# run-house/kubetorch

Hardware: AMD Instinct MI355X
Metric: llama3_8b_ddp_bf16_tokens_per_sec (higher is better)
Workload: dtype bf16; 1 GPU; model=llama3-8b, global_batch=4, seq_len=4096, parallelism=dp1

## Files before the change

kubetorch_amd/models/llama.py:

```python
from dataclasses import dataclass

import torch
import torch.nn as nn
import torch.nn.functional as F

from kubetorch_amd import ops


@dataclass
class LlamaConfig:
    dim: int = 4096
    n_layers: int = 32
    n_heads: int = 32
    n_kv_heads: int = 8
    intermediate: int = 14336
    vocab_size: int = 128256
    max_seq_len: int = 8192
    rope_base: float = 500000.0
    norm_eps: float = 1e-5
    init_std: float = 0.02

    @property
    def head_dim(self):
        return self.dim // self.n_heads
# ... 57 lines not shown
        if P == 0:
            o = layer.attn._sdpa(q, kf, vf, causal=True)
        elif S == 1:
            o = layer.attn._sdpa(q, kf, vf)
        else:
            L = P + S
            ar = torch.arange(L, device=q.device)
            mask = (ar.view(1, L) <= (P + torch.arange(
                S, device=q.device)).view(S, 1)).view(1, 1, S, L)
            o = layer.attn._sdpa(q, kf, vf, mask=mask)
        return o.transpose(1, 2).reshape(B, S, -1)


class RMSNorm(nn.Module):
    def __init__(self, dim, eps):
        super().__init__()
        self.weight = nn.Parameter(torch.ones(dim))
        self.eps = eps

    def forward(self, x):
        return ops.rmsnorm(x, self.weight, self.eps)


class Attention(nn.Module):
    def __init__(self, cfg: LlamaConfig):
        super().__init__()
        self.cfg = cfg
        d, hd = cfg.dim, cfg.head_dim
        self.n_heads, self.n_kv = cfg.n_heads, cfg.n_kv_heads
        self.wqkv = ops.Linear(d, (cfg.n_heads + 2 * cfg.n_kv_heads) * hd, bias=False)
        self.wo = ops.Linear(cfg.n_heads * hd, d, bias=False)

    def _sdpa(self, q, k, v, causal=False, mask=None):
        kw = dict(attn_mask=mask, is_causal=causal)
        if self.n_kv != self.n_heads:
            try:
                return F.scaled_dot_product_attention(
                    q, k, v, enable_gqa=True, **kw)
            except (TypeError, RuntimeError):
                rep = self.n_heads // self.n_kv
                k = k.repeat_interleave(rep, dim=1)
                v = v.repeat_interleave(rep, dim=1)
        return F.scaled_dot_product_attention(q, k, v, **kw)

    def forward(self, x, cos, sin):
        import os

        B, S, _ = x.shape
        hd = self.cfg.head_dim
        qkv = self.wqkv(x)
        q, k, v = qkv.split(
            [self.n_heads * hd, self.n_kv * hd, self.n_kv * hd], dim=-1
        )
        attn_impl = os.environ.get("KT_ATTN", "ck")
        use_v3 = (attn_impl == "ck"
                  and ops.flash_attention_v3_supported(S, hd, x.device, x.dtype))
        q_oscale = (hd ** -0.5) * ops.LOG2E if use_v3 else 1.0
        q = ops.rope(q.view(B, S, self.n_heads, hd), cos, sin, oscale=q_oscale)
        k = ops.rope(k.view(B, S, self.n_kv, hd), cos, sin)
        v = v.view(B, S, self.n_kv, hd)
        q, k, v = (t.transpose(1, 2) for t in (q, k, v))
        if use_v3:
            o = ops.flash_attention(q, k, v, impl="v3")
            return self.wo(o.transpose(1, 2).reshape(B, S, -1))
        if (attn_impl in ("ck", "custom")
                and ops.flash_attention_supported(q, k, v, True)):
            o = ops.flash_attention(
                q, k, v, impl="wmma" if attn_impl == "custom" else "ck")
            return self.wo(o.transpose(1, 2).reshape(B, S, -1))
        o = self._sdpa(q, k, v, causal=True)
        o = o.transpose(1, 2).reshape(B, S, -1)
        return self.wo(o)


class MLP(nn.Module):
    def __init__(self, cfg: LlamaConfig):
        super().__init__()
        self.w_gate_up = ops.Linear(cfg.dim, 2 * cfg.intermediate, bias=False)
        self.w_down = ops.Linear(cfg.intermediate, cfg.dim, bias=False)

    def forward(self, x):
        return self.w_down(ops.swiglu(self.w_gate_up(x)))


class Block(nn.Module):
    def __init__(self, cfg: LlamaConfig):
        super().__init__()
        self.attn_norm = RMSNorm(cfg.dim, cfg.norm_eps)
        self.attn = Attention(cfg)
        self.mlp_norm = RMSNorm(cfg.dim, cfg.norm_eps)
        self.mlp = MLP(cfg)

    def forward(self, x, cos, sin):
        x = x + self.attn(self.attn_norm(x), cos, sin)
        x = x + self.mlp(self.mlp_norm(x))
        return x


class Llama(nn.Module):
    def __init__(self, cfg: LlamaConfig):
        super().__init__()
        self.cfg = cfg
        self.embed = nn.Embedding(cfg.vocab_size, cfg.dim)
        self.layers = nn.ModuleList(Block(cfg) for _ in range(cfg.n_layers))
        self.norm = RMSNorm(cfg.dim, cfg.norm_eps)
        self.lm_head = ops.Linear(cfg.dim, cfg.vocab_size, bias=False)
        cos, sin = ops.precompute_rope(cfg.max_seq_len, cfg.head_dim, cfg.rope_base)
        self.register_buffer("rope_cos", cos, persistent=False)
        self.register_buffer("rope_sin", sin, persistent=False)
        self.gradient_checkpointing = False
        self.reset_parameters()

    def gradient_checkpointing_enable(self, enabled=True):
        self.gradient_checkpointing = enabled
        return self

    def _apply(self, fn, recurse=True):
        ret = super()._apply(fn, recurse)
        if self.rope_cos.dtype != torch.float32:
            cos, sin = ops.precompute_rope(
                self.cfg.max_seq_len, self.cfg.head_dim, self.cfg.rope_base,
# ... 115 lines not shown
```

kubetorch_amd/ops/__init__.py:

```python
import importlib.util
import os

import torch

_EXT = None
_EXT_ERR = None


def _ext():
    global _EXT, _EXT_ERR
    if _EXT is not None:
        return _EXT
    if _EXT_ERR is not None:
        raise _EXT_ERR
    so = os.path.join(os.path.dirname(__file__), "_hip_ops.so")
    if not os.path.exists(so):
        _EXT_ERR = RuntimeError(
            f"kubetorch_amd HIP extension not built: {so} missing. "
            "Run `python -m kubetorch_amd.ops.build` (gfx950)."
        )
        raise _EXT_ERR
    spec = importlib.util.spec_from_file_location("kubetorch_amd.ops._hip_ops", so)
    mod = importlib.util.module_from_spec(spec)
    try:
# ... 193 lines not shown
        du = do * g * sig
        return torch.cat([dg, du], dim=-1).to(gu.dtype)


def swiglu(gate_up):
    return _SwiGLU.apply(gate_up)


class _FusedCE(torch.autograd.Function):
    @staticmethod
    def forward(ctx, logits, targets, ignore_index):
        V = logits.shape[-1]
        flat = logits.reshape(-1, V)
        t = targets.reshape(-1)
        n_valid = (t != ignore_index).sum().clamp(min=1)
        if logits.is_cuda:
            loss = _ext().cross_entropy_fwd_(flat, t.contiguous(), 1.0, ignore_index)
            dlogits = flat
        else:
            lf = flat.float()
            logp = torch.log_softmax(lf, dim=-1)
            loss = torch.nn.functional.nll_loss(
                logp, t, reduction="none", ignore_index=ignore_index
            )
            dlogits = torch.softmax(lf, dim=-1)
            valid = (t != ignore_index).unsqueeze(-1)
            dlogits.scatter_add_(
                1, t.clamp(min=0).unsqueeze(1), -torch.ones_like(t, dtype=torch.float32).unsqueeze(1)
            )
            dlogits = torch.where(valid, dlogits, torch.zeros_like(dlogits)).to(logits.dtype)
        ctx.save_for_backward(dlogits, n_valid)
        ctx.shape = logits.shape
        return loss.sum() / n_valid.to(loss.dtype)

    @staticmethod
    def backward(ctx, gout):
        dlogits, n_valid = ctx.saved_tensors
        scale = (gout / n_valid).to(torch.float32)
        if dlogits.is_cuda:
            g = _ext().scale_bf16(dlogits, scale.reshape(1))
        else:
            g = (dlogits * scale).to(dlogits.dtype)
        return g.reshape(ctx.shape), None, None


def fused_cross_entropy(logits, targets, ignore_index=-100):
    return _FusedCE.apply(logits, targets, ignore_index)


_LN2 = 0.6931471805599453
LOG2E = 1.4426950408889634


class _FlashAttention(torch.autograd.Function):
    @staticmethod
    def forward(ctx, q, k, v, scale, impl):
        if impl == "v3":
            o, lse = _ext().attn_fwd_v3(q, k, v, scale, prescaled=True)
            scale = _LN2
        elif impl == "ck":
            o, lse = _ext().attn_fwd_ck_tr(q, k, v, scale)
        else:
            q, k, v = q.contiguous(), k.contiguous(), v.contiguous()
            o, lse = _ext().attn_fwd(q, k, v, scale)
        ctx.save_for_backward(q, k, v, o, lse)
        ctx.scale = scale
        return o

    @staticmethod
    def backward(ctx, grad_out):
        import os

        q, k, v, o, lse = ctx.saved_tensors
        B, Hq, S, D = q.shape
        Hkv = k.shape[1]
        g = Hq // Hkv
        if os.environ.get("KT_ATTN_BWD") == "ck" and S % 128 == 0:
            dq, dk_e, dv_e = _ext().attn_bwd_ck(
                grad_out.contiguous(), q.contiguous(), k.contiguous(),
                v.contiguous(), o.contiguous(), lse.contiguous(), ctx.scale)
            if g > 1:
                dk = dk_e.view(B, Hkv, g, S, D).sum(2)
                dv = dv_e.view(B, Hkv, g, S, D).sum(2)
            else:
                dk, dv = dk_e, dv_e
            return dq, dk, dv, None, None
        if g > 1:
            k_exp = k.repeat_interleave(g, dim=1)
            v_exp = v.repeat_interleave(g, dim=1)
        else:
            k_exp, v_exp = k, v
        seed = torch.zeros((), dtype=torch.long, device=q.device)
        offset = torch.zeros((), dtype=torch.long, device=q.device)
        dq, dk, dv, _ = torch.ops.aten._scaled_dot_product_efficient_attention_backward(
            grad_out.contiguous(), q, k_exp, v_exp, None, o, lse, seed, offset,
            0.0, [True, True, True, False], True, scale=ctx.scale,
        )
        if g > 1:
            dk = dk.view(B, Hkv, g, S, D).sum(2)
            dv = dv.view(B, Hkv, g, S, D).sum(2)
        return dq, dk, dv, None, None


def flash_attention(q, k, v, scale=None, impl="ck"):
    if scale is None:
        scale = q.shape[-1] ** -0.5
    return _FlashAttention.apply(q, k, v, scale, impl)


def flash_attention_supported(q, k, v, is_causal):
    return (is_causal and q.is_cuda and q.dtype == torch.bfloat16
            and q.shape[-1] == 128 and q.shape[2] % 128 == 0
            and q.shape[2] >= 256 and hip_available())


def flash_attention_v3_supported(S, head_dim, device, dtype):
    return (head_dim == 128 and S % 256 == 0 and S >= 256
            and device.type == "cuda" and dtype == torch.bfloat16
            and hip_available())


PAGED_PAGE_SIZES = (16, 32, 64)
PAGED_HEAD_DIMS = (64, 128)
PAGED_GROUPS = (1, 2, 4, 8)


def _no_grad_inputs(name, *tensors):
    if any(t.requires_grad for t in tensors):
        raise RuntimeError(f"{name} is inference-only: an input requires grad")


def _check_pools(k_pages, v_pages):
    if k_pages.dim() != 4 or v_pages.shape != k_pages.shape:
        raise ValueError("k_pages/v_pages must be equal-shaped "
                         "[num_pages, n_kv, page_size, hd]")
    if not (k_pages.is_contiguous() and v_pages.is_contiguous()):
        raise ValueError("k_pages/v_pages must be contiguous")
    if k_pages.shape[2] not in PAGED_PAGE_SIZES:
        raise ValueError(f"page_size must be one of {PAGED_PAGE_SIZES}")
    if k_pages.shape[3] not in PAGED_HEAD_DIMS:
        raise ValueError(f"head_dim must be one of {PAGED_HEAD_DIMS}")


def paged_kv_write(k_new, v_new, k_pages, v_pages, slot_mapping):
    _no_grad_inputs("paged_kv_write", k_new, v_new, k_pages, v_pages)
    if k_pages.is_cuda:
        _ext().paged_kv_write(k_new, v_new, k_pages, v_pages, slot_mapping)
        return
    _check_pools(k_pages, v_pages)
    P, Hkv, ps, hd = k_pages.shape
    if (k_new.shape != v_new.shape or k_new.dim() != 3
            or tuple(k_new.shape[1:]) != (Hkv, hd)):
        raise ValueError("k_new/v_new must be [T, n_kv, hd] matching the pool")
    if slot_mapping.dtype != torch.int32 or \
            tuple(slot_mapping.shape) != (k_new.shape[0],):
        raise ValueError("slot_mapping must be [T] int32")
    slots = slot_mapping.long()
    keep = (slots >= 0) & (slots < P * ps)
    page, off = slots[keep] // ps, slots[keep] % ps
    k_pages[page, :, off] = k_new[keep].to(k_pages.dtype)
    v_pages[page, :, off] = v_new[keep].to(v_pages.dtype)


_PAGED_TARGET_WORKGROUPS = 512
_PAGED_MIN_TOKENS_PER_SPLIT = 256
_PAGED_MAX_SPLITS = 32


def paged_num_splits(batch, n_kv, max_tokens):
    want = -(-_PAGED_TARGET_WORKGROUPS // max(1, batch * n_kv))
    cap = max(1, max_tokens // _PAGED_MIN_TOKENS_PER_SPLIT)
    return max(1, min(want, cap, _PAGED_MAX_SPLITS))
# ... 367 lines not shown
```

kubetorch_amd/ops/hip/bindings.cpp:

```cpp

#include <cmath>
#include <cstdlib>

#include <torch/extension.h>

#include <ATen/hip/impl/HIPGuardImplMasqueradingAsCUDA.h>
#include <ATen/hip/impl/HIPStreamMasqueradingAsCUDA.h>

extern "C" {
void kt_rmsnorm_fwd(const void* x, const void* res, const void* w, void* y,
                    void* s_out, void* invrms, int N, int H, float eps,
                    hipStream_t stream);
void kt_rmsnorm_bwd(const void* dy, const void* ds, const void* x,
                    const void* w, const void* invrms, void* dx,
                    void* dw_partial, void* dw, int P, int N, int H,
                    hipStream_t stream);
void kt_rope(const void* x, void* o, const void* cost, const void* sint,
             long total_quads, int S, int Hh, int D, long src_t_stride,
             long src_h_stride, float sign, float oscale, hipStream_t stream);
void kt_swiglu_fwd(const void* gu, void* out, long N, int I,
                   hipStream_t stream);
void kt_swiglu_bwd(const void* dout, const void* gu, void* dgu, long N, int I,
                   hipStream_t stream);
void kt_cross_entropy_fwd(void* logits, const void* targets, void* loss,
                          int N, int V, float scale, long ignore_index,
                          hipStream_t stream);
void kt_scale_bf16(const void* in, void* out, const void* scale, long n,
                   hipStream_t stream);
void kt_adamw(void* p, const void* g, void* m, void* v, long n, float lr,
              float beta1, float beta2, float eps, float wd, float bc1,
              float bc2, float grad_scale, hipStream_t stream);
void kt_attn_fwd(const void* q, const void* k, const void* v, void* o,
                 void* lse, int B, int Hq, int Hkv, int S, float scale,
                 hipStream_t stream);
void kt_attn_fwd_ck(const void* q, const void* k, const void* v, void* o,
                    void* lse, int B, int Hq, int Hkv, int S, float scale,
                    const long* strides, hipStream_t stream);
void kt_attn_fwd_ck_tr(const void* q, const void* k, const void* v, void* o,
                       void* lse, int B, int Hq, int Hkv, int S, float scale,
                       const long* strides, hipStream_t stream);
void kt_attn_fwd_v3(const void* q, const void* k, const void* v, void* o,
                    void* lse, int B, int Hq, int Hkv, int S, float scale,
                    const long* strides, hipStream_t stream);
void kt_pack_segments(const void* ptrs, const void* nbytes, const void* offs,
                      void* base, int nseg, long max_nbytes, int to_base,
                      hipStream_t stream);
void kt_transpose_bf16(const void* src, long src_stride, void* dst, long R,
                       long C, hipStream_t stream);
void kt_transpose_segments_bf16(const void* src, void* dst, const void* table,
                                int nseg, long max_tiles, hipStream_t stream);
void kt_attn_bwd_ck(const void* q, const void* k, const void* v,
                    const void* o, const void* do_, const void* lse, void* d,
                    void* dq_acc, void* dq, void* dk, void* dv, int B, int Hq,
                    int Hkv, int S, float scale, int mask_mode, int pipe,
                    hipStream_t stream);
void kt_paged_kv_write(const void* k_new, const void* v_new, void* k_pages,
                       void* v_pages, const void* slot_mapping, long T,
                       int Hkv, int hd, int page_size, long num_pages,
                       long k_st, long k_sh, long v_st, long v_sh,
                       hipStream_t stream);
int kt_paged_attention_decode(const void* q, const void* k_pages,
                              const void* v_pages, const void* block_table,
                              const void* seq_lens, void* out, void* po,
                              void* pm, void* pl, int B, int Hq, int Hkv,
                              int hd, int page_size, int num_pages,
                              int max_blocks, int num_splits, float scale,
                              hipStream_t stream);
int kt_paged_attention_prefill(const void* q, const void* k_pages,
                               const void* v_pages, const void* block_table,
                               const void* cu_q_lens, const void* seq_lens,
                               void* out, long T, long q_st, long q_sh, int B,
                               int Hq, int Hkv, int hd, int page_size,
// ... 47 lines not shown
  CHECK_BF16_CONTIG(dy);
  CHECK_BF16_CONTIG(x);
  CHECK_BF16_CONTIG(w);
  const int H = (int)x.size(-1);
  const long N = x.numel() / H;
  TORCH_CHECK(H % 8 == 0, "H must be a multiple of 8");
  TORCH_CHECK(w.numel() == H, "weight shape mismatch");
  TORCH_CHECK(dy.sizes() == x.sizes(), "dy shape mismatch");
  TORCH_CHECK(invrms.is_cuda() && invrms.scalar_type() == at::kFloat &&
                  invrms.is_contiguous() && invrms.numel() == N,
              "invrms must be N contiguous fp32 values on GPU");
  int lds_max = 0;
  TORCH_CHECK(hipDeviceGetAttribute(&lds_max,
                                    hipDeviceAttributeMaxSharedMemoryPerBlock,
                                    x.device().index()) == hipSuccess,
              "cannot read the LDS limit");
  TORCH_CHECK((size_t)H * sizeof(float) + 64 <= (size_t)lds_max,
              "H too large for the rmsnorm_bwd LDS accumulator");
  c10::hip::OptionalHIPGuardMasqueradingAsCUDA guard(x.device());
  auto dx = at::empty_like(x);
  auto dw = at::empty_like(w);
  const int P = N < 512 ? (int)N : 512;
  auto dw_partial = at::empty({P, H}, x.options().dtype(at::kFloat));
  const void* ds_ptr = nullptr;
  if (ds.has_value()) {
    CHECK_BF16_CONTIG(ds.value());
    TORCH_CHECK(ds->sizes() == x.sizes(), "ds shape mismatch");
    ds_ptr = ds->data_ptr();
  }
  kt_rmsnorm_bwd(dy.data_ptr(), ds_ptr, x.data_ptr(), w.data_ptr(),
                 invrms.data_ptr(), dx.data_ptr(), dw_partial.data_ptr(),
                 dw.data_ptr(), P, (int)N, H, cur_stream(x));
  return {dx, dw};
}

at::Tensor rope(const at::Tensor& x, const at::Tensor& cost,
                const at::Tensor& sint, int64_t S, double sign,
                double oscale) {
  TORCH_CHECK(x.is_cuda() && x.scalar_type() == at::kBFloat16);
  TORCH_CHECK(x.dim() == 3, "rope expects [T, Hh, D]");
  TORCH_CHECK(x.stride(2) == 1, "head dim must be contiguous");
  TORCH_CHECK(cost.scalar_type() == at::kFloat && cost.is_contiguous());
  const int D = (int)x.size(2);
  const int Hh = (int)x.size(1);
  TORCH_CHECK(D % 8 == 0, "head dim must be a multiple of 8");
  TORCH_CHECK(cost.size(0) >= S && cost.size(1) == D / 2, "cos table shape");
  c10::hip::OptionalHIPGuardMasqueradingAsCUDA guard(x.device());
  auto o = at::empty(x.sizes(), x.options());
  const long total_quads = (long)x.size(0) * Hh * (D / 8);
  kt_rope(x.data_ptr(), o.data_ptr(), cost.data_ptr(), sint.data_ptr(),
          total_quads, (int)S, Hh, D, x.stride(0), x.stride(1), (float)sign,
          (float)oscale, cur_stream(x));
  return o;
}

at::Tensor swiglu_fwd(const at::Tensor& gu) {
  CHECK_BF16_CONTIG(gu);
  const int twoI = (int)gu.size(-1);
  TORCH_CHECK(twoI % 16 == 0, "2*I must be a multiple of 16");
  const int I = twoI / 2;
  const long N = gu.numel() / twoI;
  c10::hip::OptionalHIPGuardMasqueradingAsCUDA guard(gu.device());
  auto sizes = gu.sizes().vec();
  sizes.back() = I;
  auto out = at::empty(sizes, gu.options());
  kt_swiglu_fwd(gu.data_ptr(), out.data_ptr(), N, I, cur_stream(gu));
  return out;
}

at::Tensor swiglu_bwd(const at::Tensor& dout, const at::Tensor& gu) {
  CHECK_BF16_CONTIG(dout);
  CHECK_BF16_CONTIG(gu);
  const int twoI = (int)gu.size(-1);
  TORCH_CHECK(twoI % 16 == 0, "2*I must be a multiple of 16");
  const int I = twoI / 2;
  const long N = gu.numel() / twoI;
  TORCH_CHECK(dout.size(-1) == I && dout.numel() == N * I,
              "dout shape mismatch");
  c10::hip::OptionalHIPGuardMasqueradingAsCUDA guard(gu.device());
  auto dgu = at::empty_like(gu);
  kt_swiglu_bwd(dout.data_ptr(), gu.data_ptr(), dgu.data_ptr(), N, I,
                cur_stream(gu));
  return dgu;
}

at::Tensor cross_entropy_fwd_(at::Tensor logits, const at::Tensor& targets,
                              double scale, int64_t ignore_index) {
  CHECK_BF16_CONTIG(logits);
  TORCH_CHECK(targets.scalar_type() == at::kLong && targets.is_contiguous());
  const int V = (int)logits.size(-1);
  const long N = logits.numel() / V;
  TORCH_CHECK(V % 8 == 0, "V must be a multiple of 8");
  TORCH_CHECK(targets.numel() == N, "targets shape mismatch");
  c10::hip::OptionalHIPGuardMasqueradingAsCUDA guard(logits.device());
  auto loss = at::empty({N}, logits.options().dtype(at::kFloat));
  kt_cross_entropy_fwd(logits.data_ptr(), targets.data_ptr(), loss.data_ptr(),
                       (int)N, V, (float)scale, ignore_index,
                       cur_stream(logits));
  return loss;
}

at::Tensor scale_bf16(const at::Tensor& x, const at::Tensor& scale) {
  CHECK_BF16_CONTIG(x);
  TORCH_CHECK(scale.is_cuda() && scale.scalar_type() == at::kFloat &&
                  scale.numel() == 1 && scale.device() == x.device(),
              "scale must be one fp32 value on x's device");
// ... 340 lines not shown
              "device");
  const int64_t B = block_table.size(0);
  TORCH_CHECK(cu_q_lens.is_cuda() && cu_q_lens.scalar_type() == at::kInt &&
                  cu_q_lens.is_contiguous() && cu_q_lens.dim() == 1 &&
                  cu_q_lens.size(0) == B + 1 &&
                  cu_q_lens.device() == q.device(),
              "cu_q_lens must be [B+1] contiguous int32 on q's device");
  TORCH_CHECK(seq_lens.is_cuda() && seq_lens.scalar_type() == at::kInt &&
                  seq_lens.is_contiguous() && seq_lens.dim() == 1 &&
                  seq_lens.size(0) == B && seq_lens.device() == q.device(),
              "seq_lens must be [B] contiguous int32 on q's device");
  const int64_t max_blocks = block_table.size(1);
  TORCH_CHECK(max_blocks * ps < (int64_t)INT32_MAX - 256,
              "max_blocks*page_size must fit int32");
  TORCH_CHECK(scale > 0 && std::isfinite(scale),
              "scale must be positive and finite");
  TORCH_CHECK(max_q_len >= 0 && max_q_len < (int64_t)INT32_MAX - 256,
              "max_q_len must be in [0, 2^31)");
  TORCH_CHECK(B <= 65535 && Hkv <= 65535, "grid too large");
  TORCH_CHECK(T * Hq * hd < (int64_t(1) << 46), "q too large");
  c10::hip::OptionalHIPGuardMasqueradingAsCUDA guard(q.device());
  auto out = at::zeros({T, Hq, hd}, q.options());
  if (T == 0 || B == 0 || max_q_len == 0) return out;
  const int rc = kt_paged_attention_prefill(
      q.data_ptr(), k_pages.data_ptr(), v_pages.data_ptr(),
      block_table.data_ptr(), cu_q_lens.data_ptr(), seq_lens.data_ptr(),
      out.data_ptr(), (long)T, (long)q.stride(0), (long)q.stride(1), (int)B,
      (int)Hq, Hkv, hd, ps, (int)num_pages, (int)max_blocks, (int)max_q_len,
      (float)scale, cur_stream(q));
  TORCH_CHECK(rc == 0, "paged_attention_prefill: no kernel for head_dim ", hd,
              " group ", G);
  return out;
}

}

PYBIND11_MODULE(TORCH_EXTENSION_NAME, mod) {
  mod.def("attn_fwd", &attn_fwd,
          "Causal GQA attention fwd (bf16, D=128) -> (o, lse)");
  mod.def("attn_fwd_ck", &attn_fwd_ck,
          "CK-tile FMHA fwd (bf16, D=128, causal, GQA) -> (o, lse)");
  mod.def("attn_fwd_ck_tr", &attn_fwd_ck_tr,
          "CK-tile FMHA fwd, gfx950 tr-load variant -> (o, lse)");
  mod.def("attn_fwd_v3", &attn_fwd_v3,
          "CK-tile FMHA v3 (AITER schedule) fwd with LSE -> (o, lse)",
          pybind11::arg("q"), pybind11::arg("k"), pybind11::arg("v"),
          pybind11::arg("scale"), pybind11::arg("prescaled") = false);
  mod.def("rmsnorm_fwd", &rmsnorm_fwd, "RMSNorm forward (bf16)");
  mod.def("rmsnorm_bwd", &rmsnorm_bwd, "RMSNorm backward (bf16)");
  mod.def("rope", &rope, "RoPE rotate-half (bf16), sign=+1 fwd / -1 bwd",
          pybind11::arg("x"), pybind11::arg("cost"), pybind11::arg("sint"),
          pybind11::arg("S"), pybind11::arg("sign"),
          pybind11::arg("oscale") = 1.0);
  mod.def("swiglu_fwd", &swiglu_fwd, "SwiGLU forward (bf16)");
  mod.def("swiglu_bwd", &swiglu_bwd, "SwiGLU backward (bf16)");
  mod.def("cross_entropy_fwd_", &cross_entropy_fwd_,
          "Fused CE: returns per-row loss, overwrites logits with grad");
  mod.def("scale_bf16", &scale_bf16,
          "bf16(x * scale), scale one fp32 value in device memory");
  mod.def("adamw_", &adamw_, "Fused AdamW on a flat bf16 bucket");
  mod.def("transpose_bf16", &transpose_bf16,
          "dst[C,R] = src[R,C]^T (bf16, LDS-tiled; src rows may be strided)");
  mod.def("transpose_segments_bf16", &transpose_segments_bf16,
          "Transpose every 2-D segment of a flat bf16 buffer in one launch");
  mod.def("pack_segments", &pack_segments,
          "One-kernel multi-tensor pack/unpack vs a flat buffer");
  mod.def("attn_bwd_ck", &attn_bwd_ck,
          "CK-tile GQA-native FMHA backward -> (dq, dk_exp, dv_exp)");
  mod.def("paged_kv_write", &paged_kv_write,
          "Scatter [T, n_kv, hd] k/v rows into paged pools by slot_mapping");
  mod.def("paged_attention_decode", &paged_attention_decode,
          "Single-token GQA attention over a block-table paged KV cache");
  mod.def("paged_attention_prefill", &paged_attention_prefill,
          "Causal GQA attention of packed query tokens over a paged KV cache");
}
```

kubetorch_amd/ops/hip/kernels.hip:

```cpp

#include <hip/hip_runtime.h>
#include <hip/hip_bf16.h>

typedef unsigned short u16;
typedef ushort vec8u __attribute__((ext_vector_type(8)));
typedef ushort vec4u __attribute__((ext_vector_type(4)));
typedef float vec4f __attribute__((ext_vector_type(4)));

#define WAVE 64

__device__ __forceinline__ float bf2f(u16 x) {
  unsigned int u = ((unsigned int)x) << 16;
  return __uint_as_float(u);
}
__device__ __forceinline__ u16 f2bf(float f) {
  unsigned int u = __float_as_uint(f);
  unsigned int rounding = 0x7fff + ((u >> 16) & 1);
  u += rounding;
  return (u16)(u >> 16);
}

__device__ __forceinline__ float block_reduce_sum(float v) {
  __shared__ float s[16];
#pragma unroll
// ... 115 lines not shown
  const int col = blockIdx.x * 4;
  if (col >= H) return;
  float a0 = 0.f, a1 = 0.f, a2 = 0.f, a3 = 0.f;
  for (int p = threadIdx.x; p < P; p += blockDim.x) {
    vec4f v = *reinterpret_cast<const vec4f*>(partial + (size_t)p * H + col);
    a0 += v[0]; a1 += v[1]; a2 += v[2]; a3 += v[3];
  }
  a0 = block_reduce_sum(a0);
  a1 = block_reduce_sum(a1);
  a2 = block_reduce_sum(a2);
  a3 = block_reduce_sum(a3);
  if (threadIdx.x == 0) {
    vec4u o;
    o[0] = f2bf(a0); o[1] = f2bf(a1); o[2] = f2bf(a2); o[3] = f2bf(a3);
    *reinterpret_cast<vec4u*>(out + col) = o;
  }
}

__global__ void rope_kernel(const u16* __restrict__ x, u16* __restrict__ o,
                            const float* __restrict__ cost,
                            const float* __restrict__ sint,
                            long total_quads, int S, int Hh, int D,
                            long src_t_stride, long src_h_stride,
                            float sign, float oscale) {
  const int half = D >> 1;
  const int quads_per_head = D >> 3;
  const long quads_per_tok = (long)Hh * quads_per_head;
  for (long q = (long)blockIdx.x * blockDim.x + threadIdx.x; q < total_quads;
       q += (long)gridDim.x * blockDim.x) {
    const long tok = q / quads_per_tok;
    const int rem = (int)(q - tok * quads_per_tok);
    const int h = rem / quads_per_head;
    const int qi = rem - h * quads_per_head;
    const int pos = (int)(tok % S);
    const size_t base = ((size_t)tok * Hh + h) * D + qi * 4;
    const size_t sbase = (size_t)tok * src_t_stride +
                         (size_t)h * src_h_stride + qi * 4;
    vec4u x1 = *reinterpret_cast<const vec4u*>(x + sbase);
    vec4u x2 = *reinterpret_cast<const vec4u*>(x + sbase + half);
    vec4f c = *reinterpret_cast<const vec4f*>(cost + (size_t)pos * half + qi * 4);
    vec4f s = *reinterpret_cast<const vec4f*>(sint + (size_t)pos * half + qi * 4);
    vec4u o1, o2;
#pragma unroll
    for (int j = 0; j < 4; ++j) {
      float a = bf2f(x1[j]), b = bf2f(x2[j]);
      o1[j] = f2bf((a * c[j] - sign * b * s[j]) * oscale);
      o2[j] = f2bf((b * c[j] + sign * a * s[j]) * oscale);
    }
    *reinterpret_cast<vec4u*>(o + base) = o1;
    *reinterpret_cast<vec4u*>(o + base + half) = o2;
  }
}

__global__ void swiglu_fwd_kernel(const u16* __restrict__ gu,
                                  u16* __restrict__ out, long N, int I) {
  const long total = N * (I >> 3);
  const int nvec = I >> 3;
  for (long t = (long)blockIdx.x * blockDim.x + threadIdx.x; t < total;
       t += (long)gridDim.x * blockDim.x) {
    const long row = t / nvec;
    const int vI = (int)(t - row * nvec);
    const size_t gbase = (size_t)row * 2 * I + vI * 8;
    vec8u g = __builtin_nontemporal_load(
        reinterpret_cast<const vec8u*>(gu + gbase));
    vec8u u = __builtin_nontemporal_load(
        reinterpret_cast<const vec8u*>(gu + gbase + I));
    vec8u o;
#pragma unroll
    for (int j = 0; j < 8; ++j) {
      float gf = bf2f(g[j]);
      float sig = 1.f / (1.f + __expf(-gf));
      o[j] = f2bf(gf * sig * bf2f(u[j]));
    }
    __builtin_nontemporal_store(
        o, reinterpret_cast<vec8u*>(out + (size_t)row * I + vI * 8));
  }
}

__global__ void swiglu_bwd_kernel(const u16* __restrict__ dout,
                                  const u16* __restrict__ gu,
                                  u16* __restrict__ dgu, long N, int I) {
  const long total = N * (I >> 3);
  const int nvec = I >> 3;
  for (long t = (long)blockIdx.x * blockDim.x + threadIdx.x; t < total;
       t += (long)gridDim.x * blockDim.x) {
    const long row = t / nvec;
    const int vI = (int)(t - row * nvec);
    const size_t gbase = (size_t)row * 2 * I + vI * 8;
    vec8u g = __builtin_nontemporal_load(
        reinterpret_cast<const vec8u*>(gu + gbase));
    vec8u u = __builtin_nontemporal_load(
        reinterpret_cast<const vec8u*>(gu + gbase + I));
    vec8u dov = __builtin_nontemporal_load(
        reinterpret_cast<const vec8u*>(dout + (size_t)row * I + vI * 8));
    vec8u dg, du;
#pragma unroll
    for (int j = 0; j < 8; ++j) {
      float gf = bf2f(g[j]);
      float uf = bf2f(u[j]);
      float dof = bf2f(dov[j]);
      float sig = 1.f / (1.f + __expf(-gf));
      float silu = gf * sig;
      dg[j] = f2bf(dof * uf * sig * (1.f + gf * (1.f - sig)));
      du[j] = f2bf(dof * silu);
    }
    __builtin_nontemporal_store(dg, reinterpret_cast<vec8u*>(dgu + gbase));
// ... 232 lines not shown
  const long nt = ((R + TR_TILE - 1) / TR_TILE) * tiles_c;
  for (long t = blockIdx.x; t < nt; t += gridDim.x) {
    transpose_tile_bf16<true>(src + so, C, dst + dofs, R, C,
                              (t / tiles_c) * TR_TILE, (t % tiles_c) * TR_TILE,
                              tile);
    __syncthreads();
  }
}

static inline int grid_for(long work, int block, int cap = 2048) {
  long g = (work + block - 1) / block;
  if (g > cap) g = cap;
  if (g < 1) g = 1;
  return (int)g;
}

extern "C" {

void kt_rmsnorm_fwd(const void* x, const void* res, const void* w, void* y,
                    void* s_out, void* invrms, int N, int H, float eps,
                    hipStream_t stream) {
  int grid = N < 2048 ? N : 2048;
  hipLaunchKernelGGL(rmsnorm_fwd_kernel, dim3(grid), dim3(256), 0, stream,
                     (const u16*)x, (const u16*)res, (const u16*)w, (u16*)y,
                     (u16*)s_out, (float*)invrms, N, H, eps);
}

void kt_rmsnorm_bwd(const void* dy, const void* ds, const void* x,
                    const void* w, const void* invrms, void* dx,
                    void* dw_partial, void* dw, int P, int N, int H,
                    hipStream_t stream) {
  int grid = N < P ? N : P;
  size_t lds = (size_t)H * sizeof(float);
  hipLaunchKernelGGL(rmsnorm_bwd_kernel, dim3(grid), dim3(256), lds, stream,
                     (const u16*)dy, (const u16*)ds, (const u16*)x,
                     (const u16*)w, (const float*)invrms, (u16*)dx,
                     (float*)dw_partial, N, H);
  int cgrid = (H + 3) / 4;
  hipLaunchKernelGGL(colsum_bf16_kernel, dim3(cgrid), dim3(256), 0, stream,
                     (const float*)dw_partial, (u16*)dw, grid, H);
}

void kt_rope(const void* x, void* o, const void* cost, const void* sint,
             long total_quads, int S, int Hh, int D, long src_t_stride,
             long src_h_stride, float sign, float oscale,
             hipStream_t stream) {
  int grid = grid_for(total_quads, 256);
  hipLaunchKernelGGL(rope_kernel, dim3(grid), dim3(256), 0, stream,
                     (const u16*)x, (u16*)o, (const float*)cost,
                     (const float*)sint, total_quads, S, Hh, D,
                     src_t_stride, src_h_stride, sign, oscale);
}

void kt_swiglu_fwd(const void* gu, void* out, long N, int I,
                   hipStream_t stream) {
  int grid = grid_for(N * (I >> 3), 256);
  hipLaunchKernelGGL(swiglu_fwd_kernel, dim3(grid), dim3(256), 0, stream,
                     (const u16*)gu, (u16*)out, N, I);
}

void kt_swiglu_bwd(const void* dout, const void* gu, void* dgu, long N, int I,
                   hipStream_t stream) {
  int grid = grid_for(N * (I >> 3), 256);
  hipLaunchKernelGGL(swiglu_bwd_kernel, dim3(grid), dim3(256), 0, stream,
                     (const u16*)dout, (const u16*)gu, (u16*)dgu, N, I);
}

void kt_cross_entropy_fwd(void* logits, const void* targets, void* loss, int N,
                          int V, float scale, long ignore_index,
                          hipStream_t stream) {
  int grid = N < 2048 ? N : 2048;
  hipLaunchKernelGGL(cross_entropy_fwd_kernel, dim3(grid), dim3(256), 0,
                     stream, (u16*)logits, (const long*)targets, (float*)loss,
                     N, V, scale, ignore_index);
}

void kt_scale_bf16(const void* in, void* out, const void* scale, long n,
                   hipStream_t stream) {
  long nvec = n >> 3;
  int grid = grid_for(nvec, 256);
  hipLaunchKernelGGL(scale_bf16_kernel, dim3(grid), dim3(256), 0, stream,
                     (const u16*)in, (u16*)out, (const float*)scale, nvec);
}

void kt_adamw(void* p, const void* g, void* m, void* v, long n, float lr,
              float beta1, float beta2, float eps, float wd, float bc1,
              float bc2, float grad_scale, hipStream_t stream) {
  long nvec = n >> 3;
  if (nvec > 0) {
    int grid = grid_for(nvec, 256);
    hipLaunchKernelGGL(adamw_kernel, dim3(grid), dim3(256), 0, stream, (u16*)p,
                       (const u16*)g, (float*)m, (float*)v, n, lr, beta1,
                       beta2, eps, wd, bc1, bc2, grad_scale);
  }
  long tail = n - (nvec << 3);
  if (tail > 0) {
    hipLaunchKernelGGL(adamw_tail_kernel, dim3(1), dim3(64), 0, stream,
                       (u16*)p, (const u16*)g, (float*)m, (float*)v, nvec << 3,
                       n, lr, beta1, beta2, eps, wd, bc1, bc2, grad_scale);
  }
}

void kt_pack_segments(const void* ptrs, const void* nbytes, const void* offs,
                      void* base, int nseg, long max_nbytes, int to_base,
                      hipStream_t stream) {
  int gx = grid_for(max_nbytes >> 4, 256, 1024);
// ... 25 lines not shown
```

Before: 21750 tokens/s.

## Fuse attention backward GQA reduction, RoPE transpose and qkv packing into one kernel

Adds a combined qkv-to-attention autograd function whose backward sends the expanded dq/dk/dv through a new HIP kernel. In one pass the kernel sums the GQA group gradients, applies the inverse RoPE with the q scale, and writes straight into the packed qkv gradient layout. This replaces separate group-sum reductions, two rope backward kernels and the split/cat concatenation in autograd. It adds a custom kernel with stride assumptions, with a reference fallback for layouts the kernel cannot take.

After: 22090 tokens/s, median of 6. +1.6%, better.

```diff
diff --git a/kubetorch_amd/models/llama.py b/kubetorch_amd/models/llama.py
--- a/kubetorch_amd/models/llama.py
+++ b/kubetorch_amd/models/llama.py
@@ -133,21 +133,23 @@
         q, k, v = qkv.split(
             [self.n_heads * hd, self.n_kv * hd, self.n_kv * hd], dim=-1
         )
+        q = q.view(B, S, self.n_heads, hd)
+        k = k.view(B, S, self.n_kv, hd)
+        v = v.view(B, S, self.n_kv, hd)
         attn_impl = os.environ.get("KT_ATTN", "ck")
         use_v3 = (attn_impl == "ck"
                   and ops.flash_attention_v3_supported(S, hd, x.device, x.dtype))
-        q_oscale = (hd ** -0.5) * ops.LOG2E if use_v3 else 1.0
-        q = ops.rope(q.view(B, S, self.n_heads, hd), cos, sin, oscale=q_oscale)
-        k = ops.rope(k.view(B, S, self.n_kv, hd), cos, sin)
-        v = v.view(B, S, self.n_kv, hd)
+        if use_v3 or (attn_impl == "ck" and ops.flash_attention_supported(
+                *(t.transpose(1, 2) for t in (q, k, v)), True)):
+            o = ops.qkv_attention(qkv, cos, sin, self.n_heads, self.n_kv,
+                                  "v3" if use_v3 else "ck")
+            return self.wo(o)
+        q = ops.rope(q, cos, sin)
+        k = ops.rope(k, cos, sin)
         q, k, v = (t.transpose(1, 2) for t in (q, k, v))
-        if use_v3:
-            o = ops.flash_attention(q, k, v, impl="v3")
-            return self.wo(o.transpose(1, 2).reshape(B, S, -1))
-        if (attn_impl in ("ck", "custom")
+        if (attn_impl == "custom"
                 and ops.flash_attention_supported(q, k, v, True)):
-            o = ops.flash_attention(
-                q, k, v, impl="wmma" if attn_impl == "custom" else "ck")
+            o = ops.flash_attention(q, k, v, impl="wmma")
             return self.wo(o.transpose(1, 2).reshape(B, S, -1))
         o = self._sdpa(q, k, v, causal=True)
         o = o.transpose(1, 2).reshape(B, S, -1)
diff --git a/kubetorch_amd/ops/__init__.py b/kubetorch_amd/ops/__init__.py
--- a/kubetorch_amd/ops/__init__.py
+++ b/kubetorch_amd/ops/__init__.py
@@ -269,50 +269,56 @@
 LOG2E = 1.4426950408889634
 
 
+def _attention_forward(q, k, v, scale, impl):
+    if impl == "v3":
+        o, lse = _ext().attn_fwd_v3(q, k, v, scale, prescaled=True)
+        scale = _LN2
+    elif impl == "ck":
+        o, lse = _ext().attn_fwd_ck_tr(q, k, v, scale)
+    else:
+        q, k, v = q.contiguous(), k.contiguous(), v.contiguous()
+        o, lse = _ext().attn_fwd(q, k, v, scale)
+    return q, k, v, o, lse, scale
+
+
+def _attention_backward_expanded(grad_out, q, k, v, o, lse, scale):
+    B, Hq, S, D = q.shape
+    g = Hq // k.shape[1]
+    if os.environ.get("KT_ATTN_BWD") == "ck" and S % 128 == 0:
+        return tuple(_ext().attn_bwd_ck(
+            grad_out.contiguous(), q.contiguous(), k.contiguous(),
+            v.contiguous(), o.contiguous(), lse.contiguous(), scale))
+    if g > 1:
+        k_exp = k.repeat_interleave(g, dim=1)
+        v_exp = v.repeat_interleave(g, dim=1)
+    else:
+        k_exp, v_exp = k, v
+    seed = torch.zeros((), dtype=torch.long, device=q.device)
+    offset = torch.zeros((), dtype=torch.long, device=q.device)
+    dq, dk_e, dv_e, _ = \
+        torch.ops.aten._scaled_dot_product_efficient_attention_backward(
+            grad_out, q, k_exp, v_exp, None, o, lse, seed, offset,
+            0.0, [True, True, True, False], True, scale=scale,
+        )
+    return dq, dk_e, dv_e
+
+
 class _FlashAttention(torch.autograd.Function):
     @staticmethod
     def forward(ctx, q, k, v, scale, impl):
-        if impl == "v3":
-            o, lse = _ext().attn_fwd_v3(q, k, v, scale, prescaled=True)
-            scale = _LN2
-        elif impl == "ck":
-            o, lse = _ext().attn_fwd_ck_tr(q, k, v, scale)
-        else:
-            q, k, v = q.contiguous(), k.contiguous(), v.contiguous()
-            o, lse = _ext().attn_fwd(q, k, v, scale)
+        q, k, v, o, lse, scale = _attention_forward(q, k, v, scale, impl)
         ctx.save_for_backward(q, k, v, o, lse)
         ctx.scale = scale
         return o
 
     @staticmethod
     def backward(ctx, grad_out):
-        import os
-
         q, k, v, o, lse = ctx.saved_tensors
         B, Hq, S, D = q.shape
         Hkv = k.shape[1]
         g = Hq // Hkv
-        if os.environ.get("KT_ATTN_BWD") == "ck" and S % 128 == 0:
-            dq, dk_e, dv_e = _ext().attn_bwd_ck(
-                grad_out.contiguous(), q.contiguous(), k.contiguous(),
-                v.contiguous(), o.contiguous(), lse.contiguous(), ctx.scale)
-            if g > 1:
-                dk = dk_e.view(B, Hkv, g, S, D).sum(2)
-                dv = dv_e.view(B, Hkv, g, S, D).sum(2)
-            else:
-                dk, dv = dk_e, dv_e
-            return dq, dk, dv, None, None
-        if g > 1:
-            k_exp = k.repeat_interleave(g, dim=1)
-            v_exp = v.repeat_interleave(g, dim=1)
-        else:
-            k_exp, v_exp = k, v
-        seed = torch.zeros((), dtype=torch.long, device=q.device)
-        offset = torch.zeros((), dtype=torch.long, device=q.device)
-        dq, dk, dv, _ = torch.ops.aten._scaled_dot_product_efficient_attention_backward(
-            grad_out.contiguous(), q, k_exp, v_exp, None, o, lse, seed, offset,
-            0.0, [True, True, True, False], True, scale=ctx.scale,
-        )
+        dq, dk, dv = _attention_backward_expanded(
+            grad_out.contiguous(), q, k, v, o, lse, ctx.scale)
         if g > 1:
             dk = dk.view(B, Hkv, g, S, D).sum(2)
             dv = dv.view(B, Hkv, g, S, D).sum(2)
@@ -335,6 +341,124 @@
     return (head_dim == 128 and S % 256 == 0 and S >= 256
             and device.type == "cuda" and dtype == torch.bfloat16
             and hip_available())
+
+
+def attn_pack_enabled():
+    return os.environ.get("KT_ATTN_PACK", "1") != "0"
+
+
+def _rope_bwd(dy, cos, sin, oscale):
+    if dy.is_cuda:
+        B, S, Hh, D = dy.shape
+        return _ext().rope(dy.reshape(B * S, Hh, D), cos, sin, S, -1.0,
+                           oscale).view(dy.shape)
+    return _rope_ref(dy, cos, sin, -1.0, oscale)
+
+
+def _attn_grad_pack_ref(dq, dk_e, dv_e, cos, sin, n_kv, q_oscale):
+    B, Hq, S, D = dq.shape
+    g = Hq // n_kv
+    if g > 1:
+        dk = dk_e.reshape(B, n_kv, g, S, D).sum(2)
+        dv = dv_e.reshape(B, n_kv, g, S, D).sum(2)
+    else:
+        dk, dv = dk_e, dv_e
+    dq = _rope_bwd(dq.transpose(1, 2), cos, sin, q_oscale)
+    dk = _rope_bwd(dk.transpose(1, 2), cos, sin, 1.0)
+    return torch.cat([dq.reshape(B, S, Hq * D), dk.reshape(B, S, n_kv * D),
+                      dv.transpose(1, 2).reshape(B, S, n_kv * D)], dim=-1)
+
+
+def _attn_grad_pack_kernel_ok(dq, dk_e, dv_e, cos, sin):
+    for t in (dq, dk_e, dv_e):
+        if not (t.is_cuda and t.dtype == torch.bfloat16
+                and t.device == dq.device and t.stride(3) == 1
+                and t.data_ptr() % 16 == 0):
+            return False
+        if any(t.shape[d] != 1 and (t.stride(d) < 0 or t.stride(d) % 8)
+               for d in range(3)):
+            return False
+    for t in (cos, sin):
+        if not (t.is_cuda and t.device == dq.device
+                and t.dtype == torch.float32 and t.is_contiguous()
+                and t.data_ptr() % 16 == 0):
+            return False
+    return dq.shape[3] % 8 == 0
+
+
+def attn_grad_pack(dq, dk_e, dv_e, cos, sin, n_kv, q_oscale=1.0):
+    if dq.dim() != 4 or dk_e.shape != dq.shape or dv_e.shape != dq.shape:
+        raise ValueError("dq, dk_e and dv_e must be equal-shaped "
+                         "[B, Hq, S, D]")
+    B, Hq, S, D = dq.shape
+    if n_kv < 1 or Hq % n_kv:
+        raise ValueError(f"Hq={Hq} is not a multiple of n_kv={n_kv}")
+    if D % 2 or cos.dim() != 2 or cos.shape != sin.shape \
+            or cos.shape[0] < S or cos.shape[1] != D // 2:
+        raise ValueError("cos/sin must be [>=S, D/2] tables")
+    if _attn_grad_pack_kernel_ok(dq, dk_e, dv_e, cos, sin):
+        return _ext().attn_grad_pack(dq, dk_e, dv_e, cos, sin, n_kv,
+                                     q_oscale)
+    return _attn_grad_pack_ref(dq, dk_e, dv_e, cos[:S], sin[:S], n_kv,
+                               q_oscale)
+
+
+def _qkv_split_rope(qkv, cos, sin, n_heads, n_kv, impl):
+    B, S, W = qkv.shape
+    hd = W // (n_heads + 2 * n_kv)
+    q, k, v = qkv.split([n_heads * hd, n_kv * hd, n_kv * hd], dim=-1)
+    q_oscale = (hd ** -0.5) * LOG2E if impl == "v3" else 1.0
+    q = rope(q.view(B, S, n_heads, hd), cos, sin, oscale=q_oscale)
+    k = rope(k.view(B, S, n_kv, hd), cos, sin)
+    v = v.view(B, S, n_kv, hd)
+    q, k, v = (t.transpose(1, 2) for t in (q, k, v))
+    return q, k, v, q_oscale
+
+
+class _QKVAttention(torch.autograd.Function):
+    @staticmethod
+    def forward(ctx, qkv, cos, sin, n_heads, n_kv, impl):
+        B, S, _ = qkv.shape
+        q, k, v, q_oscale = _qkv_split_rope(qkv, cos, sin, n_heads, n_kv,
+                                            impl)
+        q, k, v, o, lse, scale = _attention_forward(
+            q, k, v, q.shape[-1] ** -0.5, impl)
+        ctx.save_for_backward(q, k, v, o, lse, cos, sin)
+        ctx.scale, ctx.q_oscale, ctx.n_kv = scale, q_oscale, n_kv
+        return o.transpose(1, 2).reshape(B, S, -1)
+
+    @staticmethod
+    def backward(ctx, grad_out):
+        q, k, v, o, lse, cos, sin = ctx.saved_tensors
+        B, Hq, S, D = q.shape
+        grad_out = grad_out.reshape(B, S, Hq, D).transpose(1, 2)
+        dq, dk_e, dv_e = _attention_backward_expanded(
+            grad_out, q, k, v, o, lse, ctx.scale)
+        dqkv = attn_grad_pack(dq, dk_e, dv_e, cos, sin, ctx.n_kv,
+                              ctx.q_oscale)
+        return dqkv, None, None, None, None, None
+
+
+def qkv_attention(qkv, cos, sin, n_heads, n_kv, impl="ck"):
+    if impl not in ("v3", "ck"):
+        raise ValueError('impl must be "v3" or "ck"')
+    if qkv.dim() != 3 or qkv.shape[-1] % (n_heads + 2 * n_kv) \
+            or n_heads % n_kv:
+        raise ValueError("qkv must be [B, S, (n_heads + 2*n_kv)*D] with "
+                         "n_heads a multiple of n_kv")
+    if qkv.is_cuda and attn_pack_enabled():
+        return _QKVAttention.apply(qkv, cos, sin, n_heads, n_kv, impl)
+    B, S, _ = qkv.shape
+    q, k, v, _ = _qkv_split_rope(qkv, cos, sin, n_heads, n_kv, impl)
+    if qkv.is_cuda:
+        o = flash_attention(q, k, v, impl=impl)
+    else:
+        g = n_heads // n_kv
+        o = torch.nn.functional.scaled_dot_product_attention(
+            q, k.repeat_interleave(g, 1), v.repeat_interleave(g, 1),
+            is_causal=True,
+            scale=_LN2 if impl == "v3" else q.shape[-1] ** -0.5)
+    return o.transpose(1, 2).reshape(B, S, -1)
 
 
 PAGED_PAGE_SIZES = (16, 32, 64)
diff --git a/kubetorch_amd/ops/hip/bindings.cpp b/kubetorch_amd/ops/hip/bindings.cpp
--- a/kubetorch_amd/ops/hip/bindings.cpp
+++ b/kubetorch_amd/ops/hip/bindings.cpp
@@ -18,6 +18,10 @@
 void kt_rope(const void* x, void* o, const void* cost, const void* sint,
              long total_quads, int S, int Hh, int D, long src_t_stride,
              long src_h_stride, float sign, float oscale, hipStream_t stream);
+void kt_attn_grad_pack(const void* dq, const void* dk, const void* dv,
+                       void* out, const void* cost, const void* sint, long B,
+                       int S, int Hq, int Hkv, int D, const long* strides,
+                       float oscale, hipStream_t stream);
 void kt_swiglu_fwd(const void* gu, void* out, long N, int I,
                    hipStream_t stream);
 void kt_swiglu_bwd(const void* dout, const void* gu, void* dgu, long N, int I,
@@ -171,6 +175,55 @@
           total_quads, (int)S, Hh, D, x.stride(0), x.stride(1), (float)sign,
           (float)oscale, cur_stream(x));
   return o;
+}
+
+at::Tensor attn_grad_pack(const at::Tensor& dq, const at::Tensor& dk_e,
+                          const at::Tensor& dv_e, const at::Tensor& cost,
+                          const at::Tensor& sint, int64_t n_kv,
+                          double q_oscale) {
+  TORCH_CHECK(dq.dim() == 4, "dq must be [B, Hq, S, D]");
+  TORCH_CHECK(dk_e.sizes() == dq.sizes() && dv_e.sizes() == dq.sizes(),
+              "dq, dk_e and dv_e must have the same shape");
+  const int64_t B = dq.size(0), Hq = dq.size(1), S = dq.size(2),
+                D = dq.size(3);
+  TORCH_CHECK(D > 0 && D % 8 == 0, "head dim must be a multiple of 8");
+  TORCH_CHECK(n_kv >= 1 && Hq % n_kv == 0, "Hq must be a multiple of n_kv");
+  long strides[9];
+  int si = 0;
+  for (const at::Tensor* t : {&dq, &dk_e, &dv_e}) {
+    TORCH_CHECK(t->is_cuda() && t->scalar_type() == at::kBFloat16,
+                "gradients must be bf16 GPU tensors");
+    TORCH_CHECK(t->device() == dq.device(), "gradients on different devices");
+    TORCH_CHECK(t->stride(3) == 1, "head dim must be contiguous");
+    for (int d = 0; d < 3; ++d) {
+      TORCH_CHECK(t->size(d) == 1 ||
+                      (t->stride(d) >= 0 && t->stride(d) % 8 == 0),
+                  "strides must be non-negative multiples of 8 elements");
+      strides[si++] = t->size(d) == 1 ? 0 : t->stride(d);
+    }
+    TORCH_CHECK(reinterpret_cast<uintptr_t>(t->data_ptr()) % 16 == 0,
+                "gradients must be 16 B aligned");
+  }
+  for (const at::Tensor* t : {&cost, &sint}) {
+    TORCH_CHECK(t->is_cuda() && t->device() == dq.device() &&
+                    t->scalar_type() == at::kFloat && t->is_contiguous() &&
+                    t->dim() == 2,
+                "cos/sin must be contiguous fp32 [>=S, D/2] GPU tables");
+    TORCH_CHECK(t->size(0) >= S && t->size(1) == D / 2, "cos/sin table shape");
+    TORCH_CHECK(reinterpret_cast<uintptr_t>(t->data_ptr()) % 16 == 0,
+                "cos/sin must be 16 B aligned");
+  }
+  TORCH_CHECK(S < (int64_t(1) << 31) &&
+                  (Hq + 2 * n_kv) * D < (int64_t(1) << 31),
+              "shape out of range");
+  c10::hip::OptionalHIPGuardMasqueradingAsCUDA guard(dq.device());
+  auto out = at::empty({B, S, (Hq + 2 * n_kv) * D}, dq.options());
+  if (out.numel() == 0) return out;
+  kt_attn_grad_pack(dq.data_ptr(), dk_e.data_ptr(), dv_e.data_ptr(),
+                    out.data_ptr(), cost.data_ptr(), sint.data_ptr(), (long)B,
+                    (int)S, (int)Hq, (int)n_kv, (int)D, strides,
+                    (float)q_oscale, cur_stream(dq));
+  return out;
 }
 
 at::Tensor swiglu_fwd(const at::Tensor& gu) {
@@ -617,6 +670,11 @@
           pybind11::arg("x"), pybind11::arg("cost"), pybind11::arg("sint"),
           pybind11::arg("S"), pybind11::arg("sign"),
           pybind11::arg("oscale") = 1.0);
+  mod.def("attn_grad_pack", &attn_grad_pack,
+          "GQA group sum + RoPE^T + qkv packing of (dq, dk_exp, dv_exp)",
+          pybind11::arg("dq"), pybind11::arg("dk_e"), pybind11::arg("dv_e"),
+          pybind11::arg("cost"), pybind11::arg("sint"), pybind11::arg("n_kv"),
+          pybind11::arg("q_oscale"));
   mod.def("swiglu_fwd", &swiglu_fwd, "SwiGLU forward (bf16)");
   mod.def("swiglu_bwd", &swiglu_bwd, "SwiGLU backward (bf16)");
   mod.def("cross_entropy_fwd_", &cross_entropy_fwd_,
diff --git a/kubetorch_amd/ops/hip/kernels.hip b/kubetorch_amd/ops/hip/kernels.hip
--- a/kubetorch_amd/ops/hip/kernels.hip
+++ b/kubetorch_amd/ops/hip/kernels.hip
@@ -191,6 +191,86 @@
   }
 }
 
+template <int V>
+__global__ void attn_grad_pack_kernel(
+    const u16* __restrict__ dq, const u16* __restrict__ dk,
+    const u16* __restrict__ dv, u16* __restrict__ out,
+    const float* __restrict__ cost, const float* __restrict__ sint,
+    long total_items, int S, int Hq, int Hkv, int D,
+    long q_sb, long q_sh, long q_ss, long k_sb, long k_sh, long k_ss,
+    long v_sb, long v_sh, long v_ss, float oscale) {
+  typedef ushort vecu __attribute__((ext_vector_type(V)));
+  const int half = D >> 1;
+  const int items_per_head = half / V;
+  const int g = Hq / Hkv;
+  const long items_per_tok = (long)(Hq + 2 * Hkv) * items_per_head;
+  for (long it = (long)blockIdx.x * blockDim.x + threadIdx.x; it < total_items;
+       it += (long)gridDim.x * blockDim.x) {
+    const long tok = it / items_per_tok;
+    const int rem = (int)(it - tok * items_per_tok);
+    const int oh = rem / items_per_head;
+    const int e = (rem - oh * items_per_head) * V;
+    const long b = tok / S;
+    const int pos = (int)(tok - b * S);
+    const u16* src;
+    long sh;
+    int n = g;
+    bool rot = true;
+    float sc = 1.f;
+    if (oh < Hq) {
+      src = dq + b * q_sb + (long)oh * q_sh + (long)pos * q_ss;
+      sh = q_sh;
+      n = 1;
+      sc = oscale;
+    } else if (oh < Hq + Hkv) {
+      src = dk + b * k_sb + (long)(oh - Hq) * g * k_sh + (long)pos * k_ss;
+      sh = k_sh;
+    } else {
+      src = dv + b * v_sb + (long)(oh - Hq - Hkv) * g * v_sh + (long)pos * v_ss;
+      sh = v_sh;
+      rot = false;
+    }
+    src += e;
+    float a[V], bb[V];
+#pragma unroll
+    for (int i = 0; i < V; ++i) a[i] = bb[i] = 0.f;
+    for (int j = 0; j < n; ++j, src += sh) {
+      vecu x1 = __builtin_nontemporal_load(reinterpret_cast<const vecu*>(src));
+      vecu x2 =
+          __builtin_nontemporal_load(reinterpret_cast<const vecu*>(src + half));
+#pragma unroll
+      for (int i = 0; i < V; ++i) {
+        a[i] += bf2f(x1[i]);
+        bb[i] += bf2f(x2[i]);
+      }
+    }
+    vecu o1, o2;
+    if (rot) {
+      const float* cp = cost + (size_t)pos * half + e;
+      const float* sp = sint + (size_t)pos * half + e;
+#pragma unroll
+      for (int i = 0; i < V; i += 4) {
+        vec4f c = *reinterpret_cast<const vec4f*>(cp + i);
+        vec4f s = *reinterpret_cast<const vec4f*>(sp + i);
+#pragma unroll
+        for (int k = 0; k < 4; ++k) {
+          o1[i + k] = f2bf((a[i + k] * c[k] + bb[i + k] * s[k]) * sc);
+          o2[i + k] = f2bf((bb[i + k] * c[k] - a[i + k] * s[k]) * sc);
+        }
+      }
+    } else {
+#pragma unroll
+      for (int i = 0; i < V; ++i) {
+        o1[i] = f2bf(a[i]);
+        o2[i] = f2bf(bb[i]);
+      }
+    }
+    u16* op = out + ((size_t)tok * (Hq + 2 * Hkv) + oh) * D + e;
+    *reinterpret_cast<vecu*>(op) = o1;
+    *reinterpret_cast<vecu*>(op + half) = o2;
+  }
+}
+
 __global__ void swiglu_fwd_kernel(const u16* __restrict__ gu,
                                   u16* __restrict__ out, long N, int I) {
   const long total = N * (I >> 3);
@@ -529,6 +609,22 @@
                      src_t_stride, src_h_stride, sign, oscale);
 }
 
+void kt_attn_grad_pack(const void* dq, const void* dk, const void* dv,
+                       void* out, const void* cost, const void* sint, long B,
+                       int S, int Hq, int Hkv, int D, const long* strides,
+                       float oscale, hipStream_t stream) {
+  const int V = (D % 16 == 0) ? 8 : 4;
+  const long total = B * S * (long)(Hq + 2 * Hkv) * ((D >> 1) / V);
+  int grid = grid_for(total, 256);
+  auto kern = V == 8 ? attn_grad_pack_kernel<8> : attn_grad_pack_kernel<4>;
+  hipLaunchKernelGGL(kern, dim3(grid), dim3(256), 0, stream, (const u16*)dq,
+                     (const u16*)dk, (const u16*)dv, (u16*)out,
+                     (const float*)cost, (const float*)sint, total, S, Hq,
+                     Hkv, D, strides[0], strides[1], strides[2], strides[3],
+                     strides[4], strides[5], strides[6], strides[7],
+                     strides[8], oscale);
+}
+
 void kt_swiglu_fwd(const void* gu, void* out, long N, int I,
                    hipStream_t stream) {
   int grid = grid_for(N * (I >> 3), 256);
```
